# omerbt/TokenFlow

Measured on NVIDIA H100. Metric: frames/sec for 40-frame 512x512 SD1.5 50-step edit, higher is better.
Workload: dtype fp16

## Files before the change

tokenflow_b200/csrc/tf_ext_attn.cu:

```cuda
#include <cmath>
#include <type_traits>

#include "tf_common.cuh"
#include "tf_kernels.h"
#include "tf_wgmma.cuh"

namespace tf {
namespace {

constexpr int kBlockM = 128;
constexpr int kMaxStages = 8;
constexpr int kSmemBudget = 227 * 1024;

struct AttnCtl {
  uint64_t q_full;
  uint64_t full[kMaxStages];
  uint64_t empty[kMaxStages];
};

struct AttnParams {
  int S, heads, d;
  int tiles_m;
  int stages;
  float scale_log2;
  long long out_tok_stride;
  int q_row0;
  int q_row_end;
  int out_rows;
};

struct Item {
  int out_u, out_c, q, k0, v_u0, v_c0, n_kv;
};
__device__ __forceinline__ Item item_of(const AttnTable& t, int i) {
  const AttnSample& s = t.s[i];
  return {s.out_sample, -1, s.q_sample, s.k_sample0, s.v_sample0, -1, s.n_kv};
}
__device__ __forceinline__ Item item_of(const AttnPairTable& t, int i) {
  const AttnPair& p = t.p[i];
  return {p.out_u, p.out_c, p.q_sample, p.k_sample0, p.v_u0, p.v_c0, p.n_kv};
}

template <int kDChunks, int kBlockN, int kNPV, class Tab>
__global__ void __launch_bounds__(256, 1)
ext_attn_kernel(const __grid_constant__ CUtensorMap map_q, const __grid_constant__ CUtensorMap map_k,
                const __grid_constant__ CUtensorMap map_v, const __grid_constant__ Tab tab, const AttnParams prm,
                __half* __restrict__ out) {
  constexpr int kNV = std::is_same<Tab, AttnPairTable>::value ? 2 : 1;
  constexpr int kQChunkBytes = kBlockM * 128;
  constexpr int kKVChunkBytes = kBlockN * 128;
  constexpr int kQBytes = kDChunks * kQChunkBytes;
  constexpr int kTileBytes = kDChunks * kKVChunkBytes;
  constexpr int kStageBytes = (1 + kNV) * kTileBytes;
  constexpr int kS = kBlockN / 2;
  constexpr int kO = kNPV / 2;
  static_assert(kNPV <= 64 * kDChunks, "P V width exceeds the loaded channels");

  extern __shared__ uint8_t smem_raw[];
  uint8_t* smem = reinterpret_cast<uint8_t*>((reinterpret_cast<uintptr_t>(smem_raw) + 1023) & ~uintptr_t(1023));
  uint8_t* q_smem = smem;
  uint8_t* ring = smem + kQBytes;
  AttnCtl* ctl = reinterpret_cast<AttnCtl*>(ring + prm.stages * kStageBytes);

  const int S = prm.S, d = prm.d, stages = prm.stages;
  const int per_sample = prm.heads * prm.tiles_m;
  const int slot = blockIdx.x / per_sample;
  const int rem = blockIdx.x - slot * per_sample;
  const int head = rem / prm.tiles_m;
  const int m0 = prm.q_row0 + (rem - head * prm.tiles_m) * kBlockM;
  const Item it = item_of(tab, slot);
  const int tiles_per_slab = (S + kBlockN - 1) / kBlockN;
  const int T = it.n_kv * tiles_per_slab;
  const int ksteps = (d + 15) / 16;

  auto load_tile = [&](int t) {
    const int st = t % stages;
    const int slab = t / tiles_per_slab;
    const int n0 = (t - slab * tiles_per_slab) * kBlockN;
    uint8_t* dst = ring + st * kStageBytes;
    mbar_arrive_expect_tx(&ctl->full[st], (uint32_t)kStageBytes);
#pragma unroll
    for (int c = 0; c < kDChunks; ++c) {
      tma_load_4d(dst + c * kKVChunkBytes, &map_k, &ctl->full[st], c * 64, head, n0, it.k0 + slab);
      tma_load_4d(dst + kTileBytes + c * kKVChunkBytes, &map_v, &ctl->full[st], c * 64, head, n0, it.v_u0 + slab);
      if (kNV == 2)
        tma_load_4d(dst + 2 * kTileBytes + c * kKVChunkBytes, &map_v, &ctl->full[st], c * 64, head, n0,
                    it.v_c0 + slab);
    }
  };

  if (threadIdx.x == 0) {
    tma_prefetch_desc(&map_q);
    tma_prefetch_desc(&map_k);
    tma_prefetch_desc(&map_v);
    mbar_init(&ctl->q_full, 1);
    for (int i = 0; i < stages; ++i) {
      mbar_init(&ctl->full[i], 1);
      mbar_init(&ctl->empty[i], 8);
    }
    fence_mbar_init();
  }
  __syncthreads();
  if (threadIdx.x == 0) {
    mbar_arrive_expect_tx(&ctl->q_full, (uint32_t)kQBytes);
#pragma unroll
    for (int c = 0; c < kDChunks; ++c) tma_load_4d(q_smem + c * kQChunkBytes, &map_q, &ctl->q_full, c * 64, head, m0, it.q);
    for (int t = 0; t < stages && t < T; ++t) load_tile(t);
  }
  __syncwarp();

  const int wg = threadIdx.x >> 7;
  const int lane = threadIdx.x & 31;
  const int wrow = ((threadIdx.x >> 5) & 3) * 16 + (lane >> 2);
  const int qcol = 2 * (lane & 3);

  float o[kNV][kO];
#pragma unroll
  for (int v = 0; v < kNV; ++v)
#pragma unroll
    for (int i = 0; i < kO; ++i) o[v][i] = 0.f;
  float m_r[2] = {-INFINITY, -INFINITY}, l_r[2] = {0.f, 0.f};
  const float sl2 = prm.scale_log2;

  const uint32_t q_addr = smem_u32(q_smem) + wg * 64 * 128;
  const uint32_t ring_addr = smem_u32(ring);
  mbar_wait(&ctl->q_full, 0);
  __syncwarp();

  for (int t = 0; t < T; ++t) {
    const int st = t % stages;
    mbar_wait(&ctl->full[st], (uint32_t)(t / stages) & 1u);
    __syncwarp();
    const uint32_t k_addr = ring_addr + st * kStageBytes;

    float s[kS];
    wgmma_fence();
    for (int kk = 0; kk < ksteps; ++kk) {
      const uint32_t off = (kk & 3) * 32;
      wgmma_ss<kBlockN>(s, wgmma_desc(q_addr + (kk >> 2) * kQChunkBytes + off, 16, 1024),
                        wgmma_desc(k_addr + (kk >> 2) * kKVChunkBytes + off, 16, 1024), kk > 0 ? 1u : 0u);
    }
    wgmma_commit();
    wgmma_wait<0>();
    reg_fence(s);

    const int n0 = (t % tiles_per_slab) * kBlockN;
    if (n0 + kBlockN > S) {
      const int valid = S - n0;
#pragma unroll
      for (int j = 0; j < kBlockN / 8; ++j) {
        const int c = 8 * j + qcol;
        if (c >= valid) { s[4 * j] = -INFINITY; s[4 * j + 2] = -INFINITY; }
        if (c + 1 >= valid) { s[4 * j + 1] = -INFINITY; s[4 * j + 3] = -INFINITY; }
      }
    }

    float mx[2] = {-INFINITY, -INFINITY};
#pragma unroll
    for (int j = 0; j < kBlockN / 8; ++j) {
      mx[0] = fmaxf(mx[0], fmaxf(s[4 * j], s[4 * j + 1]));
      mx[1] = fmaxf(mx[1], fmaxf(s[4 * j + 2], s[4 * j + 3]));
    }
    float corr[2], mneg[2];
#pragma unroll
    for (int r = 0; r < 2; ++r) {
      mx[r] = fmaxf(mx[r], __shfl_xor_sync(0xffffffffu, mx[r], 1));
      mx[r] = fmaxf(mx[r], __shfl_xor_sync(0xffffffffu, mx[r], 2));
      const float m_new = fmaxf(m_r[r], mx[r] * sl2);
      corr[r] = fast_exp2(m_r[r] - m_new);
      m_r[r] = m_new;
      mneg[r] = -m_new;
      l_r[r] *= corr[r];
    }
    uint32_t pa[kBlockN / 16][4];
#pragma unroll
    for (int j = 0; j < kBlockN / 8; ++j) {
      const float p0 = fast_exp2(fmaf(s[4 * j], sl2, mneg[0]));
      const float p1 = fast_exp2(fmaf(s[4 * j + 1], sl2, mneg[0]));
      const float p2 = fast_exp2(fmaf(s[4 * j + 2], sl2, mneg[1]));
      const float p3 = fast_exp2(fmaf(s[4 * j + 3], sl2, mneg[1]));
      l_r[0] += p0 + p1;
      l_r[1] += p2 + p3;
      pa[j >> 1][(j & 1) * 2 + 0] = pack_f16x2_rn(p0, p1);
      pa[j >> 1][(j & 1) * 2 + 1] = pack_f16x2_rn(p2, p3);
    }
#pragma unroll
    for (int v = 0; v < kNV; ++v)
#pragma unroll
      for (int j = 0; j < kO / 4; ++j) {
        o[v][4 * j] *= corr[0]; o[v][4 * j + 1] *= corr[0];
        o[v][4 * j + 2] *= corr[1]; o[v][4 * j + 3] *= corr[1];
      }

#pragma unroll
    for (int v = 0; v < kNV; ++v) reg_fence(o[v]);
    wgmma_fence();
#pragma unroll
    for (int kk = 0; kk < kBlockN / 16; ++kk)
#pragma unroll
      for (int v = 0; v < kNV; ++v)
        wgmma_rs<kNPV>(o[v], pa[kk], wgmma_desc(k_addr + (1 + v) * kTileBytes + kk * 16 * 128, kKVChunkBytes, 1024), 1u);
    wgmma_commit();
    wgmma_wait<0>();
#pragma unroll
    for (int v = 0; v < kNV; ++v) reg_fence(o[v]);

    __syncwarp();
    if (lane == 0) mbar_arrive(&ctl->empty[st]);
    if (threadIdx.x == 0 && t >= 1 && t - 1 + stages < T) {
      const int pt = t - 1;
      mbar_wait(&ctl->empty[pt % stages], (uint32_t)(pt / stages) & 1u);
      load_tile(pt + stages);
    }
    __syncwarp();
  }

#pragma unroll
  for (int r = 0; r < 2; ++r) {
    l_r[r] += __shfl_xor_sync(0xffffffffu, l_r[r], 1);
    l_r[r] += __shfl_xor_sync(0xffffffffu, l_r[r], 2);
    l_r[r] = 1.f / l_r[r];
  }
#pragma unroll
  for (int v = 0; v < kNV; ++v) {
    const int out_slab = v == 0 ? it.out_u : it.out_c;
#pragma unroll
    for (int r = 0; r < 2; ++r) {
      const int tok = m0 + wg * 64 + wrow + 8 * r;
      if (tok >= prm.q_row_end) continue;
      __half* dst = out + ((long long)out_slab * prm.out_rows + (tok - prm.q_row0)) * prm.out_tok_stride + head * d;
#pragma unroll
      for (int j = 0; j < kO / 4; ++j) {
        const int c = 8 * j + qcol;
        if (c < d)
          *reinterpret_cast<uint32_t*>(dst + c) = pack_f16x2_rn(o[v][4 * j + 2 * r] * l_r[r], o[v][4 * j + 2 * r + 1] * l_r[r]);
      }
    }
  }
}

template <int kDChunks, int kBlockN, int kNPV, class Tab>
int launch_cfg(const void* q, const void* k, const void* v, long long q_tok_stride, long long kv_tok_stride,
               int q_samples_total, int kv_samples_total, const Tab& tab, int n_items, int S, int heads, int d,
               float scale, void* out, int q_row0, int q_nrows, cudaStream_t stream) {
  constexpr int kNV = std::is_same<Tab, AttnPairTable>::value ? 2 : 1;
  constexpr int kQBytes = kDChunks * kBlockM * 128;
  constexpr int kStageBytes = (1 + kNV) * kDChunks * kBlockN * 128;
  int stages = (kSmemBudget - 2048 - kQBytes) / kStageBytes;
  if (stages > kMaxStages) stages = kMaxStages;
  if (stages < 2) { set_last_error("tf_ext_attn: configuration does not fit shared memory"); return TF_ERR_UNSUPPORTED; }
  const size_t smem_bytes = 1024 + kQBytes + (size_t)stages * kStageBytes + sizeof(AttnCtl);

  CUtensorMap map_q, map_k, map_v;
  auto make = [&](CUtensorMap* m, const void* base, long long tok_stride, int samples, int box_rows) -> int {
    const uint64_t dims[4] = {(uint64_t)d, (uint64_t)heads, (uint64_t)S, (uint64_t)samples};
    const uint64_t strides[3] = {(uint64_t)d * 2, (uint64_t)tok_stride * 2, (uint64_t)S * tok_stride * 2};
    const uint32_t box[4] = {64, 1, (uint32_t)box_rows, 1};
    CUresult r = encode_tiled(m, CU_TENSOR_MAP_DATA_TYPE_FLOAT16, 4, base, dims, strides, box,
                              CU_TENSOR_MAP_SWIZZLE_128B);
    if (r != CUDA_SUCCESS) { set_last_error("tf_ext_attn: cuTensorMapEncodeTiled failed: %d", (int)r); return TF_ERR_DRIVER; }
    return TF_OK;
  };
  if (int e = make(&map_q, q, q_tok_stride, q_samples_total, kBlockM)) return e;
  if (int e = make(&map_k, k, kv_tok_stride, kv_samples_total, kBlockN)) return e;
  if (int e = make(&map_v, v, kv_tok_stride, kv_samples_total, kBlockN)) return e;

  AttnParams prm;
  prm.S = S; prm.heads = heads; prm.d = d;
  prm.q_row0 = q_row0; prm.q_row_end = (q_row0 + q_nrows < S) ? q_row0 + q_nrows : S; prm.out_rows = q_nrows;
  prm.tiles_m = (prm.q_row_end - q_row0 + kBlockM - 1) / kBlockM;
  prm.stages = stages;
  prm.scale_log2 = scale * 1.4426950408889634f;
  prm.out_tok_stride = (long long)heads * d;

  auto kern = ext_attn_kernel<kDChunks, kBlockN, kNPV, Tab>;
  if (check_cuda(cudaFuncSetAttribute(kern, cudaFuncAttributeMaxDynamicSharedMemorySize, (int)smem_bytes),
                 "tf_ext_attn smem attribute"))
    return TF_ERR_CUDA;
  const long long grid = (long long)n_items * heads * prm.tiles_m;
  kern<<<(unsigned)grid, 256, smem_bytes, stream>>>(map_q, map_k, map_v, tab, prm, static_cast<__half*>(out));
  return check_cuda(cudaGetLastError(), "tf_ext_attn launch");
}

template <class Tab>
int dispatch(const void* q, const void* k, const void* v, long long q_tok_stride, long long kv_tok_stride,
             int q_samples_total, int kv_samples_total, const Tab& tab, int n_items, int S, int heads, int d,
             float scale, void* out, int q_row0, int q_nrows, cudaStream_t stream) {
  constexpr bool kPair = std::is_same<Tab, AttnPairTable>::value;
#define TF_CFG(C, N, P)                                                                                          \
  case P:                                                                                                       \
    if constexpr (!kPair || P <= 64)                                                                            \
      return launch_cfg<C, N, P, Tab>(q, k, v, q_tok_stride, kv_tok_stride, q_samples_total, kv_samples_total,  \
                                      tab, n_items, S, heads, d, scale, out, q_row0, q_nrows, stream);          \
    break
  switch ((d + 15) / 16 * 16) {
    TF_CFG(1, 128, 16); TF_CFG(1, 128, 32); TF_CFG(1, 128, 48); TF_CFG(1, 128, 64);
    TF_CFG(2, 128, 80); TF_CFG(2, 128, 96); TF_CFG(2, 128, 112); TF_CFG(2, 128, 128);
    TF_CFG(3, 64, 144); TF_CFG(3, 64, 160); TF_CFG(3, 64, 176); TF_CFG(3, 64, 192);
    default: break;
  }
#undef TF_CFG
  set_last_error("tf_ext_attn: head dim %d > 192 is not supported", d);
  return TF_ERR_UNSUPPORTED;
}

}

int launch_ext_attn(const void* q, const void* k, const void* v, long long q_tok_stride, long long kv_tok_stride,
                    int q_samples_total, int kv_samples_total, const AttnTable& tab, int n_out, int S, int heads,
                    int d, float scale, void* out, int q_row0, int q_nrows, cudaStream_t stream) {
  if (n_out == 0 || S == 0 || q_nrows <= 0 || q_row0 >= S) return TF_OK;
  return dispatch(q, k, v, q_tok_stride, kv_tok_stride, q_samples_total, kv_samples_total, tab, n_out, S, heads, d,
                  scale, out, q_row0, q_nrows, stream);
}

bool ext_attn_pairs_supported(int d) {
  return d <= 64;
}

int launch_ext_attn_pairs(const void* q, const void* k, const void* v, long long q_tok_stride, long long kv_tok_stride,
                          int q_samples_total, int kv_samples_total, const AttnPairTable& tab, int n_pairs, int S,
                          int heads, int d, float scale, void* out, int q_row0, int q_nrows, cudaStream_t stream) {
  if (n_pairs == 0 || S == 0 || q_nrows <= 0 || q_row0 >= S) return TF_OK;
  if (!ext_attn_pairs_supported(d)) {
    set_last_error("tf_ext_attn: paired kernel does not cover d=%d", d);
    return TF_ERR_UNSUPPORTED;
  }
  return dispatch(q, k, v, q_tok_stride, kv_tok_stride, q_samples_total, kv_samples_total, tab, n_pairs, S, heads, d,
                  scale, out, q_row0, q_nrows, stream);
}

}
```

tokenflow_b200/csrc/tf_common.cuh:

```cuda
#pragma once

#include <cuda.h>
#include <cuda_fp16.h>
#include <cuda_runtime.h>
#include <stdint.h>
#include <stdio.h>

namespace tf {

void set_last_error(const char* fmt, ...);
int  check_cuda(cudaError_t e, const char* what);

enum Status : int {
  TF_OK = 0,
  TF_ERR_INVALID_ARGUMENT = 1,
  TF_ERR_CUDA = 2,
  TF_ERR_UNSUPPORTED = 3,
  TF_ERR_DRIVER = 4,
};

CUresult encode_tiled(CUtensorMap* map, CUtensorMapDataType dtype, uint32_t rank, const void* base,
                      const uint64_t* dims, const uint64_t* strides_bytes ,
                      const uint32_t* box, CUtensorMapSwizzle swizzle);

int sm_count();

#ifdef __CUDACC__
__device__ __forceinline__ uint32_t smem_u32(const void* p) {
  return static_cast<uint32_t>(__cvta_generic_to_shared(p));
}
__device__ __forceinline__ uint32_t lane_id() { return threadIdx.x & 31u; }

__device__ __forceinline__ void mbar_init(uint64_t* bar, uint32_t count) {
  asm volatile("mbarrier.init.shared::cta.b64 [%0], %1;" ::"r"(smem_u32(bar)), "r"(count) : "memory");
}
__device__ __forceinline__ void fence_mbar_init() {
  asm volatile("fence.mbarrier_init.release.cluster;" ::: "memory");
}
__device__ __forceinline__ void mbar_arrive(uint64_t* bar) {
  asm volatile("mbarrier.arrive.shared::cta.b64 _, [%0];" ::"r"(smem_u32(bar)) : "memory");
}
__device__ __forceinline__ void mbar_arrive_expect_tx(uint64_t* bar, uint32_t bytes) {
  asm volatile("mbarrier.arrive.expect_tx.shared::cta.b64 _, [%0], %1;" ::"r"(smem_u32(bar)), "r"(bytes)
               : "memory");
}
__device__ __forceinline__ bool mbar_try_wait(uint64_t* bar, uint32_t parity) {
  uint32_t ok;
  asm volatile(
      "{\n\t.reg .pred p;\n\t"
      "mbarrier.try_wait.parity.shared::cta.b64 p, [%1], %2;\n\t"
      "selp.u32 %0, 1, 0, p;\n\t}\n"
      : "=r"(ok)
      : "r"(smem_u32(bar)), "r"(parity)
      : "memory");
  return ok != 0;
}
__device__ __forceinline__ uint64_t global_timer_ns() {
  uint64_t t;
  asm volatile("mov.u64 %0, %%globaltimer;" : "=l"(t));
  return t;
}
__device__ __forceinline__ void mbar_wait(uint64_t* bar, uint32_t parity) {
  uint32_t spins = 0;
  uint64_t t0 = 0;
  while (!mbar_try_wait(bar, parity)) {
    if ((++spins & 2047u) == 0) {
      const uint64_t now = global_timer_ns();
      if (t0 == 0) t0 = now;
      if (now - t0 > 2000000000ull) __trap();
    }
  }
}

__device__ __forceinline__ void tma_prefetch_desc(const CUtensorMap* m) {
  asm volatile("prefetch.tensormap [%0];" ::"l"(reinterpret_cast<uint64_t>(m)) : "memory");
}
__device__ __forceinline__ void tma_load_3d(void* smem_dst, const CUtensorMap* m, uint64_t* bar, int c0,
                                            int c1, int c2) {
  asm volatile(
      "cp.async.bulk.tensor.3d.shared::cluster.global.tile.mbarrier::complete_tx::bytes"
      " [%0], [%1, {%3, %4, %5}], [%2];"
      ::"r"(smem_u32(smem_dst)), "l"(reinterpret_cast<uint64_t>(m)), "r"(smem_u32(bar)), "r"(c0), "r"(c1),
      "r"(c2)
      : "memory");
}
__device__ __forceinline__ void tma_load_4d(void* smem_dst, const CUtensorMap* m, uint64_t* bar, int c0,
                                            int c1, int c2, int c3) {
  asm volatile(
      "cp.async.bulk.tensor.4d.shared::cluster.global.tile.mbarrier::complete_tx::bytes"
      " [%0], [%1, {%3, %4, %5, %6}], [%2];"
      ::"r"(smem_u32(smem_dst)), "l"(reinterpret_cast<uint64_t>(m)), "r"(smem_u32(bar)), "r"(c0), "r"(c1),
      "r"(c2), "r"(c3)
      : "memory");
}

__device__ __forceinline__ uint64_t wgmma_desc(uint32_t smem_addr, uint32_t lbo_bytes, uint32_t sbo_bytes) {
  uint64_t d = 0;
  d |= static_cast<uint64_t>((smem_addr & 0x3FFFFu) >> 4);
  d |= static_cast<uint64_t>((lbo_bytes >> 4) & 0x3FFFu) << 16;
  d |= static_cast<uint64_t>((sbo_bytes >> 4) & 0x3FFFu) << 32;
  d |= static_cast<uint64_t>(1) << 62;
  return d;
}
__device__ __forceinline__ void wgmma_fence() { asm volatile("wgmma.fence.sync.aligned;" ::: "memory"); }
__device__ __forceinline__ void wgmma_commit() { asm volatile("wgmma.commit_group.sync.aligned;" ::: "memory"); }
template <int kPending>
__device__ __forceinline__ void wgmma_wait() {
  asm volatile("wgmma.wait_group.sync.aligned %0;" ::"n"(kPending) : "memory");
}
template <int N>
__device__ __forceinline__ void reg_fence(float (&r)[N]) {
#pragma unroll
  for (int i = 0; i < N; ++i) asm volatile("" : "+f"(r[i])::"memory");
}

__device__ __forceinline__ uint32_t pack_f16x2_rn(float lo, float hi) {
  uint32_t r;
  asm("cvt.rn.f16x2.f32 %0, %1, %2;" : "=r"(r) : "f"(hi), "f"(lo));
  return r;
}
__device__ __forceinline__ float fast_exp2(float x) {
  float y;
  asm("ex2.approx.ftz.f32 %0, %1;" : "=f"(y) : "f"(x));
  return y;
}
#endif

}
```

Measured before the change: 2.915.

## Overlap P·V wgmma of previous tile with QK^T of next tile in extended attention

```diff
diff --git a/tokenflow_b200/csrc/tf_ext_attn.cu b/tokenflow_b200/csrc/tf_ext_attn.cu
--- a/tokenflow_b200/csrc/tf_ext_attn.cu
+++ b/tokenflow_b200/csrc/tf_ext_attn.cu
@@ -41,7 +41,7 @@
   return {p.out_u, p.out_c, p.q_sample, p.k_sample0, p.v_u0, p.v_c0, p.n_kv};
 }
 
-template <int kDChunks, int kBlockN, int kNPV, class Tab>
+template <int kDChunks, int kBlockN, int kNPV, bool kPipe, class Tab>
 __global__ void __launch_bounds__(256, 1)
 ext_attn_kernel(const __grid_constant__ CUtensorMap map_q, const __grid_constant__ CUtensorMap map_k,
                 const __grid_constant__ CUtensorMap map_v, const __grid_constant__ Tab tab, const AttnParams prm,
@@ -71,7 +71,6 @@
   const Item it = item_of(tab, slot);
   const int tiles_per_slab = (S + kBlockN - 1) / kBlockN;
   const int T = it.n_kv * tiles_per_slab;
-  const int ksteps = (d + 15) / 16;
 
   auto load_tile = [&](int t) {
     const int st = t % stages;
@@ -127,92 +126,213 @@
   mbar_wait(&ctl->q_full, 0);
   __syncwarp();
 
-  for (int t = 0; t < T; ++t) {
-    const int st = t % stages;
-    mbar_wait(&ctl->full[st], (uint32_t)(t / stages) & 1u);
-    __syncwarp();
-    const uint32_t k_addr = ring_addr + st * kStageBytes;
-
-    float s[kS];
-    wgmma_fence();
-    for (int kk = 0; kk < ksteps; ++kk) {
-      const uint32_t off = (kk & 3) * 32;
-      wgmma_ss<kBlockN>(s, wgmma_desc(q_addr + (kk >> 2) * kQChunkBytes + off, 16, 1024),
-                        wgmma_desc(k_addr + (kk >> 2) * kKVChunkBytes + off, 16, 1024), kk > 0 ? 1u : 0u);
+  if constexpr (!kPipe) {
+    const int ksteps = (d + 15) / 16;
+    for (int t = 0; t < T; ++t) {
+      const int st = t % stages;
+      mbar_wait(&ctl->full[st], (uint32_t)(t / stages) & 1u);
+      __syncwarp();
+      const uint32_t k_addr = ring_addr + st * kStageBytes;
+
+      float s[kS];
+      wgmma_fence();
+      for (int kk = 0; kk < ksteps; ++kk) {
+        const uint32_t off = (kk & 3) * 32;
+        wgmma_ss<kBlockN>(s, wgmma_desc(q_addr + (kk >> 2) * kQChunkBytes + off, 16, 1024),
+                          wgmma_desc(k_addr + (kk >> 2) * kKVChunkBytes + off, 16, 1024), kk > 0 ? 1u : 0u);
+      }
+      wgmma_commit();
+      wgmma_wait<0>();
+      reg_fence(s);
+
+      const int n0 = (t % tiles_per_slab) * kBlockN;
+      if (n0 + kBlockN > S) {
+        const int valid = S - n0;
+#pragma unroll
+        for (int j = 0; j < kBlockN / 8; ++j) {
+          const int c = 8 * j + qcol;
+          if (c >= valid) { s[4 * j] = -INFINITY; s[4 * j + 2] = -INFINITY; }
+          if (c + 1 >= valid) { s[4 * j + 1] = -INFINITY; s[4 * j + 3] = -INFINITY; }
+        }
+      }
+
+      float mx[2] = {-INFINITY, -INFINITY};
+#pragma unroll
+      for (int j = 0; j < kBlockN / 8; ++j) {
+        mx[0] = fmaxf(mx[0], fmaxf(s[4 * j], s[4 * j + 1]));
+        mx[1] = fmaxf(mx[1], fmaxf(s[4 * j + 2], s[4 * j + 3]));
+      }
+      float corr[2], mneg[2];
+#pragma unroll
+      for (int r = 0; r < 2; ++r) {
+        mx[r] = fmaxf(mx[r], __shfl_xor_sync(0xffffffffu, mx[r], 1));
+        mx[r] = fmaxf(mx[r], __shfl_xor_sync(0xffffffffu, mx[r], 2));
+        const float m_new = fmaxf(m_r[r], mx[r] * sl2);
+        corr[r] = fast_exp2(m_r[r] - m_new);
+        m_r[r] = m_new;
+        mneg[r] = -m_new;
+        l_r[r] *= corr[r];
+      }
+      uint32_t pa[kBlockN / 16][4];
+#pragma unroll
+      for (int j = 0; j < kBlockN / 8; ++j) {
+        const float p0 = fast_exp2(fmaf(s[4 * j], sl2, mneg[0]));
+        const float p1 = fast_exp2(fmaf(s[4 * j + 1], sl2, mneg[0]));
+        const float p2 = fast_exp2(fmaf(s[4 * j + 2], sl2, mneg[1]));
+        const float p3 = fast_exp2(fmaf(s[4 * j + 3], sl2, mneg[1]));
+        l_r[0] += p0 + p1;
+        l_r[1] += p2 + p3;
+        pa[j >> 1][(j & 1) * 2 + 0] = pack_f16x2_rn(p0, p1);
+        pa[j >> 1][(j & 1) * 2 + 1] = pack_f16x2_rn(p2, p3);
+      }
+#pragma unroll
+      for (int v = 0; v < kNV; ++v)
+#pragma unroll
+        for (int j = 0; j < kO / 4; ++j) {
+          o[v][4 * j] *= corr[0]; o[v][4 * j + 1] *= corr[0];
+          o[v][4 * j + 2] *= corr[1]; o[v][4 * j + 3] *= corr[1];
+        }
+
+#pragma unroll
+      for (int v = 0; v < kNV; ++v) reg_fence(o[v]);
+      wgmma_fence();
+#pragma unroll
+      for (int kk = 0; kk < kBlockN / 16; ++kk)
+#pragma unroll
+        for (int v = 0; v < kNV; ++v)
+          wgmma_rs<kNPV>(o[v], pa[kk], wgmma_desc(k_addr + (1 + v) * kTileBytes + kk * 16 * 128, kKVChunkBytes, 1024), 1u);
+      wgmma_commit();
+      wgmma_wait<0>();
+#pragma unroll
+      for (int v = 0; v < kNV; ++v) reg_fence(o[v]);
+
+      __syncwarp();
+      if (lane == 0) mbar_arrive(&ctl->empty[st]);
+      if (threadIdx.x == 0 && t >= 1 && t - 1 + stages < T) {
+        const int pt = t - 1;
+        mbar_wait(&ctl->empty[pt % stages], (uint32_t)(pt / stages) & 1u);
+        load_tile(pt + stages);
+      }
+      __syncwarp();
     }
-    wgmma_commit();
+
+  } else {
+    auto issue_pv = [&](const uint32_t (&pa)[kBlockN / 16][4], int t) {
+      const uint32_t v_addr = ring_addr + (t % stages) * kStageBytes + kTileBytes;
+      wgmma_fence();
+#pragma unroll
+      for (int kk = 0; kk < kBlockN / 16; ++kk)
+#pragma unroll
+        for (int v = 0; v < kNV; ++v)
+          wgmma_rs<kNPV>(o[v], pa[kk], wgmma_desc(v_addr + v * kTileBytes + kk * 16 * 128, kKVChunkBytes, 1024), 1u);
+      wgmma_commit();
+    };
+
+    uint32_t p_even[kBlockN / 16][4], p_odd[kBlockN / 16][4];
+    auto iteration = [&](int t, bool first, const uint32_t (&pa)[kBlockN / 16][4], uint32_t (&pn)[kBlockN / 16][4]) {
+      const int st = t % stages;
+      mbar_wait(&ctl->full[st], (uint32_t)(t / stages) & 1u);
+      __syncwarp();
+      const uint32_t k_addr = ring_addr + st * kStageBytes;
+
+      float s[kS];
+#pragma unroll
+      for (int v = 0; v < kNV; ++v) reg_fence(o[v]);
+      wgmma_fence();
+#pragma unroll
+      for (int kk = 0; kk < kNPV / 16; ++kk) {
+        const uint32_t off = (kk & 3) * 32;
+        wgmma_ss<kBlockN>(s, wgmma_desc(q_addr + (kk >> 2) * kQChunkBytes + off, 16, 1024),
+                          wgmma_desc(k_addr + (kk >> 2) * kKVChunkBytes + off, 16, 1024), kk > 0 ? 1u : 0u);
+      }
+      wgmma_commit();
+      if (!first) {
+        issue_pv(pa, t - 1);
+        wgmma_wait<1>();
+      } else {
+        wgmma_wait<0>();
+      }
+      reg_fence(s);
+
+      const int n0 = (t % tiles_per_slab) * kBlockN;
+      if (n0 + kBlockN > S) {
+        const int valid = S - n0;
+#pragma unroll
+        for (int j = 0; j < kBlockN / 8; ++j) {
+          const int c = 8 * j + qcol;
+          if (c >= valid) { s[4 * j] = -INFINITY; s[4 * j + 2] = -INFINITY; }
+          if (c + 1 >= valid) { s[4 * j + 1] = -INFINITY; s[4 * j + 3] = -INFINITY; }
+        }
+      }
+
+      float mx[2] = {-INFINITY, -INFINITY};
+#pragma unroll
+      for (int j = 0; j < kBlockN / 8; ++j) {
+        mx[0] = fmaxf(mx[0], fmaxf(s[4 * j], s[4 * j + 1]));
+        mx[1] = fmaxf(mx[1], fmaxf(s[4 * j + 2], s[4 * j + 3]));
+      }
+      float corr[2], mneg[2];
+#pragma unroll
+      for (int r = 0; r < 2; ++r) {
+        mx[r] = fmaxf(mx[r], __shfl_xor_sync(0xffffffffu, mx[r], 1));
+        mx[r] = fmaxf(mx[r], __shfl_xor_sync(0xffffffffu, mx[r], 2));
+        const float m_new = fmaxf(m_r[r], mx[r] * sl2);
+        corr[r] = fast_exp2(m_r[r] - m_new);
+        m_r[r] = m_new;
+        mneg[r] = -m_new;
+        l_r[r] *= corr[r];
+      }
+#pragma unroll
+      for (int j = 0; j < kBlockN / 8; ++j) {
+        const float p0 = fast_exp2(fmaf(s[4 * j], sl2, mneg[0]));
+        const float p1 = fast_exp2(fmaf(s[4 * j + 1], sl2, mneg[0]));
+        const float p2 = fast_exp2(fmaf(s[4 * j + 2], sl2, mneg[1]));
+        const float p3 = fast_exp2(fmaf(s[4 * j + 3], sl2, mneg[1]));
+        l_r[0] += p0 + p1;
+        l_r[1] += p2 + p3;
+        pn[j >> 1][(j & 1) * 2 + 0] = pack_f16x2_rn(p0, p1);
+        pn[j >> 1][(j & 1) * 2 + 1] = pack_f16x2_rn(p2, p3);
+      }
+
+      wgmma_wait<0>();
+#pragma unroll
+      for (int v = 0; v < kNV; ++v) {
+        reg_fence(o[v]);
+#pragma unroll
+        for (int j = 0; j < kO / 4; ++j) {
+          o[v][4 * j] *= corr[0]; o[v][4 * j + 1] *= corr[0];
+          o[v][4 * j + 2] *= corr[1]; o[v][4 * j + 3] *= corr[1];
+        }
+      }
+      if (!first) {
+        __syncwarp();
+        if (lane == 0) mbar_arrive(&ctl->empty[(t - 1) % stages]);
+        if (threadIdx.x == 0 && t >= 2 && t - 2 + stages < T) {
+          const int pt = t - 2;
+          mbar_wait(&ctl->empty[pt % stages], (uint32_t)(pt / stages) & 1u);
+          load_tile(pt + stages);
+        }
+        __syncwarp();
+      }
+    };
+    iteration(0, true, p_odd, p_even);
+    for (int t = 1; t < T; t += 2) {
+      iteration(t, false, p_even, p_odd);
+      if (t + 1 < T) iteration(t + 1, false, p_odd, p_even);
+    }
+    uint32_t pl[kBlockN / 16][4];
+    const bool last_odd = (T - 1) & 1;
+#pragma unroll
+    for (int kk = 0; kk < kBlockN / 16; ++kk)
+#pragma unroll
+      for (int i = 0; i < 4; ++i) pl[kk][i] = last_odd ? p_odd[kk][i] : p_even[kk][i];
+#pragma unroll
+    for (int v = 0; v < kNV; ++v) reg_fence(o[v]);
+    issue_pv(pl, T - 1);
     wgmma_wait<0>();
-    reg_fence(s);
-
-    const int n0 = (t % tiles_per_slab) * kBlockN;
-    if (n0 + kBlockN > S) {
-      const int valid = S - n0;
-#pragma unroll
-      for (int j = 0; j < kBlockN / 8; ++j) {
-        const int c = 8 * j + qcol;
-        if (c >= valid) { s[4 * j] = -INFINITY; s[4 * j + 2] = -INFINITY; }
-        if (c + 1 >= valid) { s[4 * j + 1] = -INFINITY; s[4 * j + 3] = -INFINITY; }
-      }
-    }
-
-    float mx[2] = {-INFINITY, -INFINITY};
-#pragma unroll
-    for (int j = 0; j < kBlockN / 8; ++j) {
-      mx[0] = fmaxf(mx[0], fmaxf(s[4 * j], s[4 * j + 1]));
-      mx[1] = fmaxf(mx[1], fmaxf(s[4 * j + 2], s[4 * j + 3]));
-    }
-    float corr[2], mneg[2];
-#pragma unroll
-    for (int r = 0; r < 2; ++r) {
-      mx[r] = fmaxf(mx[r], __shfl_xor_sync(0xffffffffu, mx[r], 1));
-      mx[r] = fmaxf(mx[r], __shfl_xor_sync(0xffffffffu, mx[r], 2));
-      const float m_new = fmaxf(m_r[r], mx[r] * sl2);
-      corr[r] = fast_exp2(m_r[r] - m_new);
-      m_r[r] = m_new;
-      mneg[r] = -m_new;
-      l_r[r] *= corr[r];
-    }
-    uint32_t pa[kBlockN / 16][4];
-#pragma unroll
-    for (int j = 0; j < kBlockN / 8; ++j) {
-      const float p0 = fast_exp2(fmaf(s[4 * j], sl2, mneg[0]));
-      const float p1 = fast_exp2(fmaf(s[4 * j + 1], sl2, mneg[0]));
-      const float p2 = fast_exp2(fmaf(s[4 * j + 2], sl2, mneg[1]));
-      const float p3 = fast_exp2(fmaf(s[4 * j + 3], sl2, mneg[1]));
-      l_r[0] += p0 + p1;
-      l_r[1] += p2 + p3;
-      pa[j >> 1][(j & 1) * 2 + 0] = pack_f16x2_rn(p0, p1);
-      pa[j >> 1][(j & 1) * 2 + 1] = pack_f16x2_rn(p2, p3);
-    }
-#pragma unroll
-    for (int v = 0; v < kNV; ++v)
-#pragma unroll
-      for (int j = 0; j < kO / 4; ++j) {
-        o[v][4 * j] *= corr[0]; o[v][4 * j + 1] *= corr[0];
-        o[v][4 * j + 2] *= corr[1]; o[v][4 * j + 3] *= corr[1];
-      }
-
 #pragma unroll
     for (int v = 0; v < kNV; ++v) reg_fence(o[v]);
-    wgmma_fence();
-#pragma unroll
-    for (int kk = 0; kk < kBlockN / 16; ++kk)
-#pragma unroll
-      for (int v = 0; v < kNV; ++v)
-        wgmma_rs<kNPV>(o[v], pa[kk], wgmma_desc(k_addr + (1 + v) * kTileBytes + kk * 16 * 128, kKVChunkBytes, 1024), 1u);
-    wgmma_commit();
-    wgmma_wait<0>();
-#pragma unroll
-    for (int v = 0; v < kNV; ++v) reg_fence(o[v]);
-
-    __syncwarp();
-    if (lane == 0) mbar_arrive(&ctl->empty[st]);
-    if (threadIdx.x == 0 && t >= 1 && t - 1 + stages < T) {
-      const int pt = t - 1;
-      mbar_wait(&ctl->empty[pt % stages], (uint32_t)(pt / stages) & 1u);
-      load_tile(pt + stages);
-    }
-    __syncwarp();
+
   }
 
 #pragma unroll
@@ -239,16 +359,16 @@
   }
 }
 
-template <int kDChunks, int kBlockN, int kNPV, class Tab>
+template <int kDChunks, int kBlockN, int kNPV, bool kPipe, class Tab>
 int launch_cfg(const void* q, const void* k, const void* v, long long q_tok_stride, long long kv_tok_stride,
                int q_samples_total, int kv_samples_total, const Tab& tab, int n_items, int S, int heads, int d,
                float scale, void* out, int q_row0, int q_nrows, cudaStream_t stream) {
   constexpr int kNV = std::is_same<Tab, AttnPairTable>::value ? 2 : 1;
   constexpr int kQBytes = kDChunks * kBlockM * 128;
   constexpr int kStageBytes = (1 + kNV) * kDChunks * kBlockN * 128;
-  int stages = (kSmemBudget - 2048 - kQBytes) / kStageBytes;
-  if (stages > kMaxStages) stages = kMaxStages;
-  if (stages < 2) { set_last_error("tf_ext_attn: configuration does not fit shared memory"); return TF_ERR_UNSUPPORTED; }
+  constexpr int kFit = (kSmemBudget - 2048 - kQBytes) / kStageBytes;
+  constexpr int stages = kFit < kMaxStages ? kFit : kMaxStages;
+  static_assert(stages >= (kPipe ? 3 : 2), "tf_ext_attn: configuration does not fit shared memory");
   const size_t smem_bytes = 1024 + kQBytes + (size_t)stages * kStageBytes + sizeof(AttnCtl);
 
   CUtensorMap map_q, map_k, map_v;
@@ -273,7 +393,7 @@
   prm.scale_log2 = scale * 1.4426950408889634f;
   prm.out_tok_stride = (long long)heads * d;
 
-  auto kern = ext_attn_kernel<kDChunks, kBlockN, kNPV, Tab>;
+  auto kern = ext_attn_kernel<kDChunks, kBlockN, kNPV, kPipe, Tab>;
   if (check_cuda(cudaFuncSetAttribute(kern, cudaFuncAttributeMaxDynamicSharedMemorySize, (int)smem_bytes),
                  "tf_ext_attn smem attribute"))
     return TF_ERR_CUDA;
@@ -287,16 +407,17 @@
              int q_samples_total, int kv_samples_total, const Tab& tab, int n_items, int S, int heads, int d,
              float scale, void* out, int q_row0, int q_nrows, cudaStream_t stream) {
   constexpr bool kPair = std::is_same<Tab, AttnPairTable>::value;
-#define TF_CFG(C, N, P)                                                                                          \
+#define TF_CFG(C, N, P, PIPE)                                                                                    \
   case P:                                                                                                       \
     if constexpr (!kPair || P <= 64)                                                                            \
-      return launch_cfg<C, N, P, Tab>(q, k, v, q_tok_stride, kv_tok_stride, q_samples_total, kv_samples_total,  \
-                                      tab, n_items, S, heads, d, scale, out, q_row0, q_nrows, stream);          \
+      return launch_cfg<C, N, P, PIPE, Tab>(q, k, v, q_tok_stride, kv_tok_stride, q_samples_total,               \
+                                            kv_samples_total, tab, n_items, S, heads, d, scale, out, q_row0,    \
+                                            q_nrows, stream);                                                   \
     break
   switch ((d + 15) / 16 * 16) {
-    TF_CFG(1, 128, 16); TF_CFG(1, 128, 32); TF_CFG(1, 128, 48); TF_CFG(1, 128, 64);
-    TF_CFG(2, 128, 80); TF_CFG(2, 128, 96); TF_CFG(2, 128, 112); TF_CFG(2, 128, 128);
-    TF_CFG(3, 64, 144); TF_CFG(3, 64, 160); TF_CFG(3, 64, 176); TF_CFG(3, 64, 192);
+    TF_CFG(1, 128, 16, true); TF_CFG(1, 128, 32, true); TF_CFG(1, 128, 48, true); TF_CFG(1, 128, 64, true);
+    TF_CFG(2, 128, 80, false); TF_CFG(2, 128, 96, false); TF_CFG(2, 128, 112, false); TF_CFG(2, 128, 128, false);
+    TF_CFG(3, 64, 144, false); TF_CFG(3, 64, 160, false); TF_CFG(3, 64, 176, false); TF_CFG(3, 64, 192, false);
     default: break;
   }
 #undef TF_CFG
```

New measurement: 2.952 (median of 6 runs). 1.01x the previous value.

## Templatize warpgroup count per head dim and fully unroll QK wgmma loop

Applied to the files above, without the earlier changes.

```diff
diff --git a/tokenflow_b200/csrc/tf_common.cuh b/tokenflow_b200/csrc/tf_common.cuh
--- a/tokenflow_b200/csrc/tf_common.cuh
+++ b/tokenflow_b200/csrc/tf_common.cuh
@@ -113,6 +113,11 @@
 #pragma unroll
   for (int i = 0; i < N; ++i) asm volatile("" : "+f"(r[i])::"memory");
 }
+template <int N>
+__device__ __forceinline__ void reg_fence(uint32_t (&r)[N]) {
+#pragma unroll
+  for (int i = 0; i < N; ++i) asm volatile("" : "+r"(r[i])::"memory");
+}
 
 __device__ __forceinline__ uint32_t pack_f16x2_rn(float lo, float hi) {
   uint32_t r;
diff --git a/tokenflow_b200/csrc/tf_ext_attn.cu b/tokenflow_b200/csrc/tf_ext_attn.cu
--- a/tokenflow_b200/csrc/tf_ext_attn.cu
+++ b/tokenflow_b200/csrc/tf_ext_attn.cu
@@ -8,7 +8,6 @@
 namespace tf {
 namespace {
 
-constexpr int kBlockM = 128;
 constexpr int kMaxStages = 8;
 constexpr int kSmemBudget = 227 * 1024;
 
@@ -41,12 +40,13 @@
   return {p.out_u, p.out_c, p.q_sample, p.k_sample0, p.v_u0, p.v_c0, p.n_kv};
 }
 
-template <int kDChunks, int kBlockN, int kNPV, class Tab>
-__global__ void __launch_bounds__(256, 1)
+template <int kDChunks, int kBlockN, int kNPV, int kWG, class Tab>
+__global__ void __launch_bounds__(kWG * 128, 1)
 ext_attn_kernel(const __grid_constant__ CUtensorMap map_q, const __grid_constant__ CUtensorMap map_k,
                 const __grid_constant__ CUtensorMap map_v, const __grid_constant__ Tab tab, const AttnParams prm,
                 __half* __restrict__ out) {
   constexpr int kNV = std::is_same<Tab, AttnPairTable>::value ? 2 : 1;
+  constexpr int kBlockM = kWG * 64;
   constexpr int kQChunkBytes = kBlockM * 128;
   constexpr int kKVChunkBytes = kBlockN * 128;
   constexpr int kQBytes = kDChunks * kQChunkBytes;
@@ -71,7 +71,6 @@
   const Item it = item_of(tab, slot);
   const int tiles_per_slab = (S + kBlockN - 1) / kBlockN;
   const int T = it.n_kv * tiles_per_slab;
-  const int ksteps = (d + 15) / 16;
 
   auto load_tile = [&](int t) {
     const int st = t % stages;
@@ -96,7 +95,7 @@
     mbar_init(&ctl->q_full, 1);
     for (int i = 0; i < stages; ++i) {
       mbar_init(&ctl->full[i], 1);
-      mbar_init(&ctl->empty[i], 8);
+      mbar_init(&ctl->empty[i], kWG * 4);
     }
     fence_mbar_init();
   }
@@ -126,21 +125,30 @@
   const uint32_t ring_addr = smem_u32(ring);
   mbar_wait(&ctl->q_full, 0);
   __syncwarp();
+  const bool active = m0 + wg * 64 < prm.q_row_end;
 
   for (int t = 0; t < T; ++t) {
     const int st = t % stages;
     mbar_wait(&ctl->full[st], (uint32_t)(t / stages) & 1u);
     __syncwarp();
+    if (!active) {
+      if (lane == 0) mbar_arrive(&ctl->empty[st]);
+      __syncwarp();
+      continue;
+    }
     const uint32_t k_addr = ring_addr + st * kStageBytes;
 
     float s[kS];
+    reg_fence(s);
     wgmma_fence();
-    for (int kk = 0; kk < ksteps; ++kk) {
+#pragma unroll
+    for (int kk = 0; kk < kNPV / 16; ++kk) {
       const uint32_t off = (kk & 3) * 32;
       wgmma_ss<kBlockN>(s, wgmma_desc(q_addr + (kk >> 2) * kQChunkBytes + off, 16, 1024),
                         wgmma_desc(k_addr + (kk >> 2) * kKVChunkBytes + off, 16, 1024), kk > 0 ? 1u : 0u);
     }
     wgmma_commit();
+    reg_fence(s);
     wgmma_wait<0>();
     reg_fence(s);
 
@@ -194,6 +202,8 @@
 
 #pragma unroll
     for (int v = 0; v < kNV; ++v) reg_fence(o[v]);
+#pragma unroll
+    for (int kk = 0; kk < kBlockN / 16; ++kk) reg_fence(pa[kk]);
     wgmma_fence();
 #pragma unroll
     for (int kk = 0; kk < kBlockN / 16; ++kk)
@@ -201,6 +211,10 @@
       for (int v = 0; v < kNV; ++v)
         wgmma_rs<kNPV>(o[v], pa[kk], wgmma_desc(k_addr + (1 + v) * kTileBytes + kk * 16 * 128, kKVChunkBytes, 1024), 1u);
     wgmma_commit();
+#pragma unroll
+    for (int v = 0; v < kNV; ++v) reg_fence(o[v]);
+#pragma unroll
+    for (int kk = 0; kk < kBlockN / 16; ++kk) reg_fence(pa[kk]);
     wgmma_wait<0>();
 #pragma unroll
     for (int v = 0; v < kNV; ++v) reg_fence(o[v]);
@@ -239,11 +253,12 @@
   }
 }
 
-template <int kDChunks, int kBlockN, int kNPV, class Tab>
+template <int kDChunks, int kBlockN, int kNPV, int kWG, class Tab>
 int launch_cfg(const void* q, const void* k, const void* v, long long q_tok_stride, long long kv_tok_stride,
                int q_samples_total, int kv_samples_total, const Tab& tab, int n_items, int S, int heads, int d,
                float scale, void* out, int q_row0, int q_nrows, cudaStream_t stream) {
   constexpr int kNV = std::is_same<Tab, AttnPairTable>::value ? 2 : 1;
+  constexpr int kBlockM = kWG * 64;
   constexpr int kQBytes = kDChunks * kBlockM * 128;
   constexpr int kStageBytes = (1 + kNV) * kDChunks * kBlockN * 128;
   int stages = (kSmemBudget - 2048 - kQBytes) / kStageBytes;
@@ -273,12 +288,12 @@
   prm.scale_log2 = scale * 1.4426950408889634f;
   prm.out_tok_stride = (long long)heads * d;
 
-  auto kern = ext_attn_kernel<kDChunks, kBlockN, kNPV, Tab>;
+  auto kern = ext_attn_kernel<kDChunks, kBlockN, kNPV, kWG, Tab>;
   if (check_cuda(cudaFuncSetAttribute(kern, cudaFuncAttributeMaxDynamicSharedMemorySize, (int)smem_bytes),
                  "tf_ext_attn smem attribute"))
     return TF_ERR_CUDA;
   const long long grid = (long long)n_items * heads * prm.tiles_m;
-  kern<<<(unsigned)grid, 256, smem_bytes, stream>>>(map_q, map_k, map_v, tab, prm, static_cast<__half*>(out));
+  kern<<<(unsigned)grid, kWG * 128, smem_bytes, stream>>>(map_q, map_k, map_v, tab, prm, static_cast<__half*>(out));
   return check_cuda(cudaGetLastError(), "tf_ext_attn launch");
 }
 
@@ -287,16 +302,17 @@
              int q_samples_total, int kv_samples_total, const Tab& tab, int n_items, int S, int heads, int d,
              float scale, void* out, int q_row0, int q_nrows, cudaStream_t stream) {
   constexpr bool kPair = std::is_same<Tab, AttnPairTable>::value;
-#define TF_CFG(C, N, P)                                                                                          \
+#define TF_CFG(C, N, P, W)                                                                                        \
   case P:                                                                                                       \
     if constexpr (!kPair || P <= 64)                                                                            \
-      return launch_cfg<C, N, P, Tab>(q, k, v, q_tok_stride, kv_tok_stride, q_samples_total, kv_samples_total,  \
+      return launch_cfg<C, N, P, W, Tab>(q, k, v, q_tok_stride, kv_tok_stride, q_samples_total, kv_samples_total,  \
                                       tab, n_items, S, heads, d, scale, out, q_row0, q_nrows, stream);          \
     break
   switch ((d + 15) / 16 * 16) {
-    TF_CFG(1, 128, 16); TF_CFG(1, 128, 32); TF_CFG(1, 128, 48); TF_CFG(1, 128, 64);
-    TF_CFG(2, 128, 80); TF_CFG(2, 128, 96); TF_CFG(2, 128, 112); TF_CFG(2, 128, 128);
-    TF_CFG(3, 64, 144); TF_CFG(3, 64, 160); TF_CFG(3, 64, 176); TF_CFG(3, 64, 192);
+    TF_CFG(1, 128, 16, kPair ? 3 : 4); TF_CFG(1, 128, 32, kPair ? 3 : 4); TF_CFG(1, 128, 48, kPair ? 3 : 4);
+    TF_CFG(1, 128, 64, 3);
+    TF_CFG(2, 128, 80, 2); TF_CFG(2, 128, 96, 2); TF_CFG(2, 128, 112, 2); TF_CFG(2, 128, 128, 2);
+    TF_CFG(3, 64, 144, 2); TF_CFG(3, 64, 160, 2); TF_CFG(3, 64, 176, 2); TF_CFG(3, 64, 192, 2);
     default: break;
   }
 #undef TF_CFG
```

Result: faster. 2.213 before, 2.252 after (median of 6 runs) (+1.8%).
